# will-rowe/hulk

Hardware: AMD Instinct MI355X
Metric: reads/sec (150bp, k=21, sketch=512) (higher is better)
Workload: dtype u64

## Files before the change

hulk_amd/csrc/hulk_api.hip:

```cpp
#include "hulk_oneshot.h"

#include <mutex>

#include <algorithm>
#include <cmath>
#include <cfloat>

using namespace hulk;

namespace {
thread_local std::string g_create_error;

uint64_t ipow(uint64_t a, uint64_t b) {
    uint64_t p = 1;
    while (b > 0) { if (b & 1) p *= a; b >>= 1; a *= a; }
    return p;
}

}

namespace hulk {
const char *err_text(int status) {
    switch (status) {
        case HULK_OK: return "";
// ... 89 lines not shown
    fq_sweep_idle();
    hulk_ctx *c = new hulk_ctx();
    c->p = p; c->B = (int32_t)bins; c->S = p.sketch_size; c->slot_begin = p.slot_begin; c->slots = p.slot_count;
    c->drift = p.decay_ratio != 1.0;
    c->scaling = p.decay_ratio > 0.0 && p.decay_ratio < 1.0;
    c->decay_weight = c->scaling ? std::exp(-p.decay_ratio) : 0.0;
    c->cms_width = (int)std::ceil(2 / 0.001);
    c->cms_depth = (int)std::ceil(std::log(1 - 0.99) / std::log(0.5));
    c->ntiles = (c->B + SCAN_TILE - 1) / SCAN_TILE;
    c->row_stride = (size_t)c->ntiles * SCAN_TILE;

#define CHK_CREATE(call) do { hipError_t e_ = (call); if (e_ != hipSuccess) { int rc_ = fail_hip(nullptr, e_, #call); hulk_destroy(c); return rc_; } } while (0)
    CHK_CREATE(hipSetDevice(p.device));
    {
        const int ord = lds_order_verified(p.device);
        if (ord < 0) { const int rc_ = fail_hip(nullptr, (hipError_t)(-ord), "LDS atomic-order self-test"); hulk_destroy(c); return rc_; }
        c->lds_order_ok = ord == 1;
        c->cms_chain = !c->lds_order_ok || (p.flags & HULK_FLAG_CMS_CHAIN) != 0;
    }
    CHK_CREATE(create_lane_stream(&c->own_stream, 0));
    c->stream = c->own_stream;
    const size_t B = (size_t)c->B, S = c->S, SL = c->slots;
    CHK_CREATE(dalloc(&c->d_state, 1));
    auto knob = [](const char *name, uint32_t field, uint32_t dflt, uint32_t lo, uint32_t hi) {
        uint32_t v = field ? field : dflt;
        if (const char *e = HULK_EXP_ENV(name)) { const long x = atol(e); if (x >= (long)lo && x <= (long)hi) v = (uint32_t)x; }
        return v;
    };
    c->T = knob("HULK_BATCH", p.batch, SCAN_BATCH_MAX, 1, SCAN_BATCH_MAX);
    const bool decay_on = p.decay_ratio > 0.0 && p.decay_ratio < 1.0;
    c->work_lanes = knob("HULK_WORK_LANES", p.work_lanes, decay_on ? 1 : 2, 1, 2);
    c->host_copy_threads = knob("HULK_HOST_COPY_THREADS", p.host_copy_threads, 4, 1, 32);
    c->no_overlap = (p.flags & HULK_FLAG_NO_OVERLAP) != 0 || HULK_EXP_ENV("HULK_NO_OVERLAP") != nullptr;
    c->shard_full = (p.flags & HULK_FLAG_SHARD_FULL) != 0 || HULK_EXP_ENV("HULK_SHARD_FULL") != nullptr;
    c->ring_n = c->T + 1;
    const size_t T = c->T, RN = c->ring_n;
    CHK_CREATE(dalloc(&c->d_hist, 2 * RN * B));
    {
        int lo = 0, hi = 0;
        CHK_CREATE(hipDeviceGetStreamPriorityRange(&lo, &hi));
        const char *pe = HULK_EXP_ENV("HULK_FLUSH_PRIORITY");
        const int prio = pe ? atoi(pe) : lo;
        CHK_CREATE(hipStreamCreateWithPriority(&c->flush_stream, hipStreamNonBlocking, prio));
    }
    CHK_CREATE(hipEventCreateWithFlags(&c->ev_binned, hipEventDisableTiming));
    CHK_CREATE(hipEventCreateWithFlags(&c->ev_flushed[0], hipEventDisableTiming));
// ... 61 lines not shown
        std::vector<double> w(S ? S : 1, 1.7976931348623157e308);
        CHK_CREATE(hipMemcpy(c->d_weights, w.data(), w.size() * 8, hipMemcpyHostToDevice));
    }
#undef CHK_CREATE
    int rc = build_chains(c);
    if (rc == HULK_OK && p.cws_source == HULK_CWS_GO_COMPAT) rc = generate_tables(c);
    if (rc == HULK_OK) rc = lanes_prereserve(c);
    if (rc == HULK_OK && hipStreamSynchronize(c->stream) != hipSuccess) rc = HULK_ERR_HIP;
    if (rc != HULK_OK) { g_create_error = c->last_error.empty() ? err_text(rc) : c->last_error; hulk_destroy(c); return rc; }
    *out = c;
    return HULK_OK;
}

void hulk_destroy(hulk_ctx *c) {
    if (!c) return;
    if (c->stream) hipStreamSynchronize(c->stream);
    if (c->own_stream) hipStreamSynchronize(c->own_stream);
    if (c->flush_stream) { hipStreamSynchronize(c->flush_stream); hipStreamDestroy(c->flush_stream); }
    if (c->ev_binned) hipEventDestroy(c->ev_binned);
    for (int i = 0; i < 2; i++) if (c->ev_flushed[i]) hipEventDestroy(c->ev_flushed[i]);
    for (auto &pr : c->prof) { hipEventDestroy(pr.a); hipEventDestroy(pr.b); }
    for (auto &m : c->marks) hipEventDestroy(m.e);
    hipFree(c->d_state); hipFree(c->d_hist); hipFree(c->d_hist_tmp);
    hipFree(c->d_meta8); hipFree(c->d_segsum); hipFree(c->d_cbase);
    hipFree(c->d_segadd); hipFree(c->d_segfac); hipFree(c->d_cstart); hipFree(c->d_sege0);
    hipFree(c->d_ctr); hipFree(c->d_pos16); hipFree(c->d_mins); hipFree(c->d_f64); hipFree(c->d_weights);
    hipFree(c->d_blkcnt); hipFree(c->d_eidx); hipFree(c->d_etot); hipFree(c->d_ctrd);
    hipFree(c->d_candA); hipFree(c->d_candB); hipFree(c->d_rcb); hipFree(c->d_rcp32); hipFree(c->d_rmm); hipFree(c->d_k32); hipFree(c->d_tilemin);
    hipFree(c->d_scanmap); hipFree(c->d_scanlist); hipFree(c->d_scanlist_n); hipFree(c->d_slotmin); hipFree(c->d_kmin32); hipFree(c->d_rext); hipFree(c->d_visited); hipFree(c->d_kminslot);
    for (auto &hs : c->hstage) {
        if (hs.ev) hipEventDestroy(hs.ev);
        if (hs.ev1) hipEventDestroy(hs.ev1);
        if (hs.h_bases) hipHostFree(hs.h_bases);
        if (hs.h_off) hipHostFree(hs.h_off);
        hipFree(hs.d_bases); hipFree(hs.d_off);
    }
    hipFree(c->d_min_slots);
    hipFree(c->mh.kmv); hipFree(c->mh.khf); hipFree(c->mh.xmin); hipFree(c->mh.fed); hipFree(c->d_mh_in);
    for (auto &ln : c->lane) {
        if (ln.stream) { hipStreamSynchronize(ln.stream); hipStreamDestroy(ln.stream); }
        hipFree(ln.d_slow_list); hipFree(ln.d_slow_count);
        hulk::MinimizerList &ml = ln.ml;
        hipFree(ml.x); hipFree(ml.slot); hipFree(ml.key); hipFree(ml.cnt); hipFree(ml.off); hipFree(ml.bsum); hipFree(ml.partial);
        hipFree(ml.nib); hipFree(ml.nib_over); hipFree(ml.dmask); hipFree(ml.dsum);
    }
    for (int i = 0; i < 2; i++) if (c->ev_heavy[i]) hipEventDestroy(c->ev_heavy[i]);
// ... 515 lines not shown
```

hulk_amd/csrc/hulk_countmin.hip:

```cpp
#include "hulk_device.h"

#include <math.h>
#include <stdlib.h>
#include <stdio.h>
#include <algorithm>
#include <mutex>

namespace hulk {
namespace {

__global__ __launch_bounds__(256) void k_count_used(const uint32_t *__restrict__ hists, DevState *st,
                                                    FlushBatch fb) {
    __shared__ unsigned red[4];
    const int t = blockIdx.y;
    const uint32_t slot = ring_slot(fb, t);
    if (blockIdx.x == 0 && t == 0 && threadIdx.x < RING_MAX) st->used[fb.parity ^ 1][threadIdx.x] = 0;
    const uint32_t *hist = hists + (size_t)slot * (size_t)fb.num_bins;
    unsigned cnt = 0;
    for (int32_t b = blockIdx.x * blockDim.x + threadIdx.x; b < fb.num_bins; b += gridDim.x * blockDim.x)
        cnt += hist[b] != 0;
    for (int off = 32; off; off >>= 1) cnt += __shfl_xor(cnt, off);
    if (lane_id() == 0) red[threadIdx.x >> 6] = cnt;
    __syncthreads();
    if (threadIdx.x == 0) {
// ... 5 lines not shown
constexpr int CMS_SEGS = 16;
inline int cms_seg_chunks(int32_t num_bins) { return ((num_bins + 63) / 64 + CMS_SEGS - 1) / CMS_SEGS; }

__device__ __forceinline__ void cms_seg_row_sums(uint32_t *lctr, const uint32_t *__restrict__ hist, const uint16_t *__restrict__ pos16,
                                                 size_t B, int64_t b0, int depth, int width, int seg_chunks) {
    const int tid = threadIdx.x, lane = tid & 63, d = tid >> 6;
    for (int i = tid; i < depth * width; i += blockDim.x) lctr[i] = 0;
    __syncthreads();
    if (d >= depth) return;
    const uint16_t *pd = pos16 + (size_t)d * B;
    for (int c0 = 0; c0 < seg_chunks; c0 += 8) {
        uint32_t h[8]; uint32_t p[8];
#pragma unroll
        for (int u = 0; u < 8; u++) {
            const int64_t b = b0 + (int64_t)(c0 + u) * 64 + lane;
            const bool ok = (c0 + u < seg_chunks) && b < (int64_t)B;
            h[u] = ok ? hist[b] : 0u; p[u] = ok ? pd[b] : 0u;
        }
#pragma unroll
        for (int u = 0; u < 8; u++) if (h[u]) atomicAdd(&lctr[d * width + p[u]], h[u]);
    }
}

__global__ __launch_bounds__(512) void k_cms_segsum(const uint32_t *__restrict__ hists,
                                                    const uint16_t *__restrict__ pos16,
                                                    uint32_t *__restrict__ segsum, int depth, int width,
                                                    int seg_chunks, const DevState *st, FlushBatch fb) {
    extern __shared__ __align__(16) unsigned char smem[];
    uint32_t *lctr = (uint32_t *)smem;
    const int seg = blockIdx.x, t = blockIdx.y, tid = threadIdx.x;
    const uint32_t gomask = batch_gomask(st, fb);
    if (!((gomask >> t) & 1u)) return;
    const size_t B = (size_t)fb.num_bins;
    cms_seg_row_sums(lctr, hists + (size_t)ring_slot(fb, t) * B, pos16, B, (int64_t)seg * seg_chunks * 64, depth, width, seg_chunks);
    __syncthreads();
    uint32_t *out = segsum + (((size_t)t * depth) * CMS_SEGS + 0) * width;
    for (int i = tid; i < depth * width; i += blockDim.x) {
        const int dd = i / width, p = i - dd * width;
        out[((size_t)dd * CMS_SEGS + seg) * width + p] = lctr[i];
    }
}

__global__ __launch_bounds__(256) void k_cms_base(const uint32_t *__restrict__ segsum,
                                                  unsigned long long *__restrict__ ctr,
                                                  unsigned long long *__restrict__ base, int depth, int width,
                                                  const DevState *st, FlushBatch fb) {
    const uint32_t gomask = batch_gomask(st, fb);
    const int i = blockIdx.x * blockDim.x + threadIdx.x;
    if (i >= depth * width) return;
    const int d = i / width, p = i - d * width;
    unsigned long long run = ctr[i];
    for (int t = 0; t < (int)fb.count; t++) {
        if (!((gomask >> t) & 1u)) continue;
        uint32_t sv[CMS_SEGS];
        const size_t at0 = (((size_t)t * depth + d) * CMS_SEGS) * width + p;
#pragma unroll
        for (int seg = 0; seg < CMS_SEGS; seg++) sv[seg] = segsum[at0 + (size_t)seg * width];
#pragma unroll
        for (int seg = 0; seg < CMS_SEGS; seg++) { base[at0 + (size_t)seg * width] = run; run += sv[seg]; }
    }
    ctr[i] = run;
}

// ... 369 lines not shown
    const size_t lds3 = (size_t)depth * width * 8 + (size_t)2 * CMS_GB * 8;
    static bool attr_set = false;
    if (!attr_set) {
        hipError_t e = hipFuncSetAttribute((const void *)k_cms_freq, hipFuncAttributeMaxDynamicSharedMemorySize, (int)lds3);
        if (e == hipSuccess) e = hipFuncSetAttribute((const void *)k_cms_freq_chain, hipFuncAttributeMaxDynamicSharedMemorySize, (int)lds3);
        if (e != hipSuccess) return e;
        attr_set = true;
    }
    prof_mark(s, "k_cms_segsum");
    hipLaunchKernelGGL(k_cms_segsum, dim3(CMS_SEGS, fb.count), dim3(512), lds1, s, d_hists, d_pos16, d_segsum, depth, width,
                       seg_chunks, st, fb);
    prof_mark(s, "k_cms_base");
    hipLaunchKernelGGL(k_cms_base, dim3((depth * width + 255) / 256), dim3(256), 0, s, d_segsum, d_ctr, d_base, depth, width, st, fb);
    if (chain) {
        prof_mark(s, "k_cms_freq_chain");
        hipLaunchKernelGGL(k_cms_freq_chain, dim3(CMS_SEGS, fb.count), dim3(512), lds3, s, d_base, d_meta8, d_hists, d_pos16, d_f64,
                           d_rcp32, depth, width, seg_chunks, row_stride, st, fb);
    }
    else {
        prof_mark(s, "k_cms_freq");
        hipLaunchKernelGGL(k_cms_freq, dim3(CMS_SEGS, fb.count), dim3(512), lds3, s, d_base, d_hists, d_pos16, d_f64,
                           d_rcp32, depth, width, seg_chunks, row_stride, st, fb);
    }
    return hipGetLastError();
}

size_t cms_binorder_entries(int depth, int width) { return (size_t)depth * CMS_SEGS * width; }

hipError_t launch_cmsd_binorder(hipStream_t s, uint32_t *d_hists, const uint16_t *d_pos16, const uint8_t *d_meta8,
                                const uint32_t *d_eidx, const uint32_t *d_etot, double *d_ctrd, double *d_segadd,
                                double *d_segfac, uint32_t *d_sege0, double *d_cstart, double *d_f64, float *d_rcp32,
                                int depth, int width, size_t row_stride, double omega, DevState *st, const FlushBatch &fb_in,
                                hipEvent_t freq_begin, hipEvent_t freq_end, bool chain_form) {
    FlushBatch fb = fb_in;
    const int seg_chunks = cms_seg_chunks(fb.num_bins);
    if (depth > 8) return hipErrorInvalidValue;
    { static const char *e = HULK_EXP_ENV("HULK_CMSD_PRIO"); fb.prio = e ? atoi(e) : CMSD_WAVE_PRIO; }
    const size_t lds1 = (size_t)depth * width * 8 + (size_t)2 * 512 * 8;
    const size_t lds3 = (size_t)depth * width * 8 + (size_t)2 * CMS_GB * 8;
    static bool attr_set = false;
    if (!attr_set) {
        hipError_t e = hipFuncSetAttribute((const void *)k_cmsd_segsum, hipFuncAttributeMaxDynamicSharedMemorySize, (int)lds1);
        if (e == hipSuccess) e = hipFuncSetAttribute((const void *)k_cmsd_freq, hipFuncAttributeMaxDynamicSharedMemorySize, (int)lds3);
        if (e == hipSuccess) e = hipFuncSetAttribute((const void *)k_cmsd_freq_chain, hipFuncAttributeMaxDynamicSharedMemorySize, (int)lds3);
        if (e != hipSuccess) return e;
        attr_set = true;
// ... 231 lines not shown
```

hulk_amd/csrc/hulk_ctx.h:

```cpp
#pragma once
#include "../../include/hulk_hip.h"
#include "hulk_internal.h"

#include <rccl/rccl.h>

#include <cstdlib>
#include <cstring>
#include <string>
#include <vector>

static inline int poison_byte() {
    static const int v = [] { const char *e = HULK_EXP_ENV("HULK_POISON"); return e ? (int)(strtol(e, nullptr, 0) & 0xff) : -1; }();
    return v;
}
static inline hipError_t poison_malloc(void **p, size_t n) {
    hipError_t e = (hipMalloc)(p, n);
    if (e == hipSuccess && poison_byte() >= 0 && n) { e = hipMemset(*p, poison_byte(), n); if (e == hipSuccess) e = hipDeviceSynchronize(); }
    return e;
}
static inline hipError_t poison_host_malloc(void **p, size_t n, unsigned flags) {
    hipError_t e = (hipHostMalloc)(p, n, flags);
    if (e == hipSuccess && poison_byte() >= 0 && n) memset(*p, poison_byte(), n);
    return e;
}
// ... 91 lines not shown
    hipEvent_t ev_long = nullptr; hipStream_t long_last_stream = nullptr; bool long_pending = false;
    const uint64_t *h_off_chunk = nullptr;
    uint64_t long_cap = 0, long_table_cap = 0;
    struct Snapshots {
        uint32_t every = 0, cap = 0;
        unsigned long long *d_mins = nullptr; double *d_weights = nullptr;
        uint64_t *h_mins = nullptr; double *h_weights = nullptr;
        std::vector<hulk_snapshot_info> info;
        uint64_t ordinal = 0;
        uint64_t recorded = 0, delivered = 0;
        uint64_t reads_at_flush = 0, reads_at_snapshot = 0;
        hulk_snapshot_fn fn = nullptr; void *user = nullptr; bool fn_failed = false;
        hulk_snapshot_panel_fn pfn = nullptr;
        bool has_fn() const { return fn || pfn; }
        struct Panel {
            uint32_t n = 0; int metric = 0, role = 0;
            double *d_mT = nullptr, *d_wT = nullptr;
            double *d_dist = nullptr, *h_dist = nullptr;
        } panel;
        struct Group { uint64_t first; uint32_t n; hipEvent_t ev; };
        std::vector<Group> groups; size_t group_head = 0;
        std::vector<hipEvent_t> free_events;
    } snap;
    uint64_t seq_count = 0, flush_index = 0;
    uint32_t T = 16, ring_n = 17, ring_base = 0;
    uint32_t bin_spectra = 0;
    bool tables_ready = false, finished = false, hist_hook_used = false;
    int sticky = HULK_OK;
    std::string last_error;
    int profiling = 0;
    std::vector<hulk::ProfileRec> prof;
    std::vector<hulk::ProfMark> marks;
};

namespace hulk {

const char *err_text(int status);
int fail(hulk_ctx *c, int status, const std::string &extra = std::string());
int fail_hip(hulk_ctx *c, hipError_t e, const char *what);
#define HIPCHK(c, call)                                             \
    do { hipError_t e_ = (call); if (e_ != hipSuccess) return hulk::fail_hip((c), e_, #call); } while (0)
template <typename T> hipError_t dalloc(T **p, size_t n) { return hipMalloc((void **)p, n ? n * sizeof(T) : sizeof(T)); }
inline bool metric_ok(int metric) { return metric == HULK_METRIC_JACCARD || metric == HULK_METRIC_WEIGHTED_JACCARD; }
inline bool pair_metric_ok(int metric) { return metric_ok(metric) || metric == HULK_METRIC_BOTTOMK; }
inline bool bottomk_size_ok(int metric, uint32_t sketch_size) { return metric != HULK_METRIC_BOTTOMK || sketch_size <= HULK_MINHASH_MAX_SKETCH; }
inline bool role_ok(int role) { return role == HULK_PANEL_ROW || role == HULK_PANEL_COLUMN; }

int build_chains(hulk_ctx *c);
int install_tables(hulk_ctx *c, const double *r, const double *cc, const double *b);
int generate_tables(hulk_ctx *c);
int ensure_tables(hulk_ctx *c);

constexpr unsigned PROFILE_EVENT_FLAGS = hipEventDisableSystemFence;
uint32_t *ring_hist(hulk_ctx *c);
int issue_flush(hulk_ctx *c, hipEvent_t gate = nullptr);
int ring_issue_own_flush(hulk_ctx *c);
hipEvent_t ring_write_event(hulk_ctx *c);
int ring_ready_for_writes(hulk_ctx *c);
int sync_all(hulk_ctx *c);
int fatal_status(hulk_ctx *c);
int bin_reads(hulk_ctx *c, const uint8_t *d_bases, const uint64_t *d_offsets, uint64_t n,
              uint32_t max_len, uint64_t bases_bytes, uint64_t interval, uint64_t fill, bool join = false);
hipStream_t lane_stream(hulk_ctx *c, int ring);
hipStream_t ring_stream(hulk_ctx *c);
int lanes_join(hulk_ctx *c);
int lanes_prereserve(hulk_ctx *c);
int stage_mark_busy(hulk_ctx *c, hulk_ctx::HostStage &hs);
int flush_kernels(hulk_ctx *c, hipStream_t s, uint32_t *hist, const FlushBatch &fb);
bool no_overlap_mode(const hulk_ctx *c);
hipStream_t flush_stream_of(hulk_ctx *c);
enum { FLUSH_EXPLICIT = 0, FLUSH_INTERVAL = 1, FLUSH_EOF = 2 };
int flush_batch(hulk_ctx *c, uint32_t count, hipStream_t dep_stream = nullptr, bool use_dep = false, bool allreduce = false,
                int closed_by = FLUSH_EXPLICIT);
int check_device_error(hulk_ctx *c);
int stage_host_reads(hulk_ctx *c, const uint8_t *bases, const uint64_t *offsets, uint64_t i0, uint64_t i1,
                     hulk_ctx::HostStage **out);
int check_host_reads(hulk_ctx *c, const uint64_t *offsets, uint64_t n, uint64_t *max_len_out);

hipError_t create_lane_stream(hipStream_t *s, int priority);
struct ProfScope {
    hulk_ctx *prev;
    explicit ProfScope(hulk_ctx *c);
    ~ProfScope();
};

int snap_plan(hulk_ctx *c, FlushBatch &fb, uint32_t count, int closed_by, uint64_t *first, uint32_t *n);
int snap_flush_issued(hulk_ctx *c, hipStream_t s, uint64_t first, uint32_t n);
int snap_deliver(hulk_ctx *c, bool wait, uint32_t *delivered = nullptr);
void snap_teardown(hulk_ctx *c);
int snap_panel_flush(hulk_ctx *c, hipStream_t s, const FlushBatch &fb);
int snap_refuse(hulk_ctx *c, const char *entry);
// ... 6 lines not shown
```

hulk_amd/csrc/hulk_cws.hip:

```cpp
#include "hulk_device.h"

#include <math.h>
#include <stdlib.h>
#include <algorithm>

namespace hulk {
namespace {

__device__ __forceinline__ float wave_min8_by_row(float (&m)[8]) {
    asm volatile("s_nop 1\n\t"
                 "v_permlane32_swap_b32 %0, %4\n\t"
                 "v_permlane32_swap_b32 %1, %5\n\t"
                 "v_permlane32_swap_b32 %2, %6\n\t"
                 "v_permlane32_swap_b32 %3, %7\n\t"
                 "v_min_f32 %0, %0, %4\n\t"
                 "v_min_f32 %2, %2, %6\n\t"
                 "v_min_f32 %1, %1, %5\n\t"
                 "v_min_f32 %3, %3, %7\n\t"
                 "v_permlane16_swap_b32 %0, %2\n\t"
                 "s_nop 0\n\t"
                 "v_permlane16_swap_b32 %1, %3\n\t"
                 "v_min_f32 %0, %0, %2\n\t"
                 "v_min_f32 %1, %1, %3\n\t"
                 "s_nop 1\n\t"
                 "v_min_f32_dpp %0, %0, %0 row_ror:8 row_mask:0xf bank_mask:0xf\n\t"
                 "v_min_f32_dpp %1, %1, %1 row_ror:8 row_mask:0xf bank_mask:0xf\n\t"
                 "s_nop 1\n\t"
                 "v_mov_b32_dpp %0, %1 quad_perm:[0,1,2,3] row_mask:0xf bank_mask:0xc\n\t"
                 "s_nop 1\n\t"
                 "v_min_f32_dpp %0, %0, %0 quad_perm:[1,0,3,2] row_mask:0xf bank_mask:0xf\n\t"
                 "s_nop 1\n\t"
                 "v_min_f32_dpp %0, %0, %0 quad_perm:[2,3,0,1] row_mask:0xf bank_mask:0xf\n\t"
                 "s_nop 1\n\t"
                 "v_min_f32_dpp %0, %0, %0 row_half_mirror row_mask:0xf bank_mask:0xf\n\t"
                 : "+v"(m[0]), "+v"(m[1]), "+v"(m[2]), "+v"(m[3]), "+v"(m[4]), "+v"(m[5]), "+v"(m[6]), "+v"(m[7]));
    return m[0];
}

__global__ __launch_bounds__(1024) void k_flush_decide(const unsigned long long *__restrict__ ctr, int ncounters,
                                                       const float *__restrict__ kminslot,
                                                       const double *__restrict__ weights, int slots, int slot_begin,
                                                       DevState *st, FlushBatch fb, int enable,
                                                       unsigned long long *seal, uint32_t seal_tag) {
    __shared__ unsigned long long red[16];
    __shared__ int anypass;
    const int tid = threadIdx.x;
    if (tid == 0) anypass = 0;
    unsigned long long m = ~0ull;
    for (int i = tid; i < ncounters; i += blockDim.x) { const unsigned long long v = ctr[i]; m = v < m ? v : m; }
    for (int off = 32; off; off >>= 1) { const unsigned long long o = __shfl_xor(m, off); m = o < m ? o : m; }
    if ((tid & 63) == 0) red[tid >> 6] = m;
    __syncthreads();
    m = red[0];
    for (int i = 1; i < 16; i++) m = red[i] < m ? red[i] : m;
    bool pass = false;
    if (enable == 2) pass = false;
    else if (!enable || m == 0) pass = true;
    else {
        const double rmax = 1.0 / (double)m;
        for (int s = tid; s < slots; s += blockDim.x) {
            const double km = (double)kminslot[s];
            const double w = weights[slot_begin + s];
            const double thr = w + 1e-5 * fabs(w) + 1e-37;
            const double bound = km < 0.0 ? km * rmax : 0.0;
            if (bound <= thr) pass = true;
        }
    }
    if (pass) atomicOr(&anypass, 1);
    __syncthreads();
    if (tid == 0) {
        if (seal) *seal = ((unsigned long long)seal_tag << 32) | (anypass ? 1ull : 0ull);
        else st->skip_exact[fb.parity] = anypass ? 0u : 1u;
    }
}
__global__ __launch_bounds__(256) void k_slot_kmin(const float *__restrict__ kmin32, float *__restrict__ kminslot, int wtiles) {
    __shared__ float red[4];
    const int slot = blockIdx.x;
    float m = INFINITY;
    for (int i = threadIdx.x; i < wtiles; i += blockDim.x) m = fminf(m, kmin32[(size_t)slot * wtiles + i]);
    for (int off = 32; off; off >>= 1) m = fminf(m, __shfl_xor(m, off));
    if ((threadIdx.x & 63) == 0) red[threadIdx.x >> 6] = m;
    __syncthreads();
    if (threadIdx.x == 0) kminslot[slot] = fminf(fminf(red[0], red[1]), fminf(red[2], red[3]));
}

__global__ __launch_bounds__(256) void k_tile_kmin(const float *__restrict__ k32, float *__restrict__ kmin32,
                                                   int ntiles, size_t row_stride) {
    const int slot = blockIdx.y, tile = blockIdx.x, wid = threadIdx.x >> 6;
    const floatx4 v = *(const floatx4 *)(k32 + (size_t)slot * row_stride + (size_t)tile * SCAN_TILE + (size_t)threadIdx.x * 4);
    float m = fminf(fminf(v.x, v.y), fminf(v.z, v.w));
    for (int off = 32; off; off >>= 1) m = fminf(m, __shfl_xor(m, off));
    if ((threadIdx.x & 63) == 0) kmin32[(size_t)slot * (size_t)(ntiles * 4) + (size_t)(tile * 4 + wid)] = m;
}
__global__ __launch_bounds__(256) void k_rcp_extrema(const float *__restrict__ rcp32, float *__restrict__ rext,
                                                     int ntiles, size_t row_stride, const DevState *st, FlushBatch fb) {
// ... 675 lines not shown
    if (grid_form) {
        const dim3 g((unsigned)(((wwords * 4 + 7) / 8) * 8 * groups));
        if (mode == 0) { prof_mark(s, "k_cws_scan"); hipLaunchKernelGGL(k_cws_scan<0>, g, dim3(1024), 0, s, d_k32, rv, d_tilemin, slots, ntiles, row_stride, st, fb, d_scanmap, wwords); }
        else if (mode == 1) { prof_mark(s, "k_cws_scan"); hipLaunchKernelGGL(k_cws_scan<1>, g, dim3(1024), 0, s, d_k32, rv, d_tilemin, slots, ntiles, row_stride, st, fb, d_scanmap, wwords); }
        else { prof_mark(s, "k_cws_scan"); hipLaunchKernelGGL(k_cws_scan<2>, g, dim3(1024), 0, s, d_k32, rv, d_tilemin, slots, ntiles, row_stride, st, fb, d_scanmap, wwords); }
    } else {
        const size_t items = (size_t)groups * wtiles;
        const dim3 g((unsigned)((std::min<size_t>(2048, (items + 3) / 4) + 7) / 8 * 8));
        if (mode == 0) { prof_mark(s, "k_cws_scan_list"); hipLaunchKernelGGL(k_cws_scan_list<0>, g, dim3(256), 0, s, d_k32, rv, d_tilemin, slots, ntiles, row_stride, st, fb, d_scanlist, d_scanlist_n); }
        else if (mode == 1) { prof_mark(s, "k_cws_scan_list"); hipLaunchKernelGGL(k_cws_scan_list<1>, g, dim3(256), 0, s, d_k32, rv, d_tilemin, slots, ntiles, row_stride, st, fb, d_scanlist, d_scanlist_n); }
        else { prof_mark(s, "k_cws_scan_list"); hipLaunchKernelGGL(k_cws_scan_list<2>, g, dim3(256), 0, s, d_k32, rv, d_tilemin, slots, ntiles, row_stride, st, fb, d_scanlist, d_scanlist_n); }
    }
    if (scan_end) { const hipError_t e = hipEventRecord(scan_end, s); if (e != hipSuccess) return e; }
    return hipGetLastError();
}

hipError_t launch_slot_kmin(hipStream_t s, const float *d_kmin32, float *d_kminslot, int slots, int ntiles) {
    hipLaunchKernelGGL(k_slot_kmin, dim3(slots), dim3(256), 0, s, d_kmin32, d_kminslot, ntiles * 4);
    return hipGetLastError();
}

hipError_t launch_flush_decide(hipStream_t s, const unsigned long long *d_ctr, int ncounters, const float *d_kminslot,
                               const double *d_weights, int slots, int slot_begin, DevState *st, const FlushBatch &fb,
                               int enable, unsigned long long *d_seal, uint32_t seal_tag) {
    prof_mark(s, "k_flush_decide");
    hipLaunchKernelGGL(k_flush_decide, dim3(1), dim3(1024), 0, s, d_ctr, ncounters, d_kminslot, d_weights, slots,
                       slot_begin, st, fb, enable, d_seal, seal_tag);
    return hipGetLastError();
}

hipError_t launch_tile_kmin(hipStream_t s, const float *d_k32, float *d_kmin32, int slots, int ntiles, size_t row_stride) {
    hipLaunchKernelGGL(k_tile_kmin, dim3(ntiles, slots), dim3(256), 0, s, d_k32, d_kmin32, ntiles, row_stride);
    return hipGetLastError();
}

hipError_t launch_cws_resolve(hipStream_t s, const double *d_rcb, const double *d_f64,
                              const float *d_tilemin, double *d_candA, int32_t *d_candB,
                              unsigned long long *d_mins, double *d_weights,
                              int slots, int slot_begin, int ntiles, const unsigned long long *d_scanmap, DevState *st,
                              const FlushBatch &fb, unsigned long long *d_snap_mins, double *d_snap_weights, uint32_t sketch_size) {
    const int merged = (scan_merge_off() || d_snap_mins) ? 0 : 1;
    if (merged) {
        prof_mark(s, "k_cws_resolve");
        hipLaunchKernelGGL(k_cws_resolve<true>, dim3(slots, 1), dim3(256), (size_t)ntiles * 4 * sizeof(float), s,
                           d_rcb, d_f64, d_tilemin, d_candA, d_candB, slots, ntiles, d_scanmap, (ntiles * 4 + 63) / 64, st, fb);
    }
    else {
        prof_mark(s, "k_cws_resolve");
        hipLaunchKernelGGL(k_cws_resolve<false>, dim3(slots, fb.count), dim3(256), (size_t)ntiles * 4 * sizeof(float), s,
                           d_rcb, d_f64, d_tilemin, d_candA, d_candB, slots, ntiles, d_scanmap, (ntiles * 4 + 63) / 64, st, fb);
// ... 89 lines not shown
```

hulk_amd/csrc/hulk_flush.hip:

```cpp
#include "hulk_ctx.h"

#include <algorithm>
#include <thread>

namespace hulk {

namespace { thread_local hulk_ctx *g_prof_ctx = nullptr; }
ProfScope::ProfScope(hulk_ctx *c) : prev(g_prof_ctx) { g_prof_ctx = (c && (c->profiling & 16)) ? c : nullptr; }
ProfScope::~ProfScope() { g_prof_ctx = prev; }
void prof_mark(hipStream_t s, const char *kernel) {
    hulk_ctx *c = g_prof_ctx;
    if (!c) return;
    ProfMark m{nullptr, kernel, s};
    if (hipEventCreateWithFlags(&m.e, PROFILE_EVENT_FLAGS) != hipSuccess) return;
    if (hipEventRecord(m.e, s) != hipSuccess) { (void)hipEventDestroy(m.e); return; }
    c->marks.push_back(m);
}

hipError_t create_lane_stream(hipStream_t *s, int priority) {
    if (const char *e = HULK_EXP_ENV("HULK_K1_CU_FREE")) {
        const int nfree = atoi(e);
        if (nfree > 0 && nfree < 256) {
            uint32_t mask[8];
            for (int i = 0; i < 8; i++) mask[i] = 0xffffffffu;
// ... 13 lines not shown
static int lane_of_ring(const hulk_ctx *c, int ring) { return (c->work_lanes > 1 && !c->no_overlap) ? ring : 0; }
hipStream_t ring_stream(hulk_ctx *c) { return lane_stream(c, lane_of_ring(c, c->cur_ring)); }

int ring_issue_own_flush(hulk_ctx *c) {
    if (c->deferred.armed && c->deferred.ring == c->cur_ring) return issue_flush(c, nullptr);
    return HULK_OK;
}
hipEvent_t ring_write_event(hulk_ctx *c) {
    if (!c->pending_flush[c->cur_ring]) return nullptr;
    c->pending_flush[c->cur_ring] = false;
    return c->ev_flushed[c->cur_ring];
}
int ring_ready_for_writes(hulk_ctx *c) {
    { const int rc = ring_issue_own_flush(c); if (rc != HULK_OK) return rc; }
    if (hipEvent_t e = ring_write_event(c)) HIPCHK(c, hipStreamWaitEvent(ring_stream(c), e, 0));
    return HULK_OK;
}

int fatal_status(hulk_ctx *c) {
    if (c->sticky == HULK_ERR_HIP || c->sticky == HULK_ERR_COMM) return fail(c, c->sticky);
    return HULK_OK;
}

int sync_all(hulk_ctx *c) {
    { const int rc = fatal_status(c); if (rc != HULK_OK) return rc; }
    { const int rc = issue_flush(c, nullptr); if (rc != HULK_OK) return rc; }
    HIPCHK(c, hipStreamSynchronize(c->stream));
    if (c->lane[1].stream) HIPCHK(c, hipStreamSynchronize(c->lane[1].stream));
    c->stagger = 1;
    HIPCHK(c, hipStreamSynchronize(c->flush_stream));
    return HULK_OK;
}

constexpr uint32_t GENERIC_XCAP_MAX = 1024;
bool pick_config(uint32_t k, uint32_t max_len, MinimizerParams &P, int &threads) {
    const uint32_t npos = max_len >= k ? max_len - k + 1 : 1;
    if (npos <= 192) { P.xcap = 192; P.tab_size = 256; threads = 256; return true; }
    P.xcap = GENERIC_XCAP_MAX; P.tab_size = 2048; threads = 64;
    return npos <= GENERIC_XCAP_MAX;
}

int bin_long_reads(hulk_ctx *c, hipStream_t s, const uint8_t *d_bases, const uint64_t *d_offsets, uint64_t n, MinimizerParams P,
                   uint32_t *hist, const uint64_t *h_offsets) {
    std::vector<uint64_t> fetched;
    const uint64_t *off = h_offsets;
    if (!off) {
        fetched.resize(n + 1);
        HIPCHK(c, hipMemcpyAsync(fetched.data(), d_offsets, (n + 1) * 8, hipMemcpyDeviceToHost, s));
        HIPCHK(c, hipStreamSynchronize(s));
        off = fetched.data();
    }
    constexpr uint64_t GROUP_POS = 128ull << 20;
    constexpr uint32_t GROUP_SEQS = 32768;
// ... 233 lines not shown
        ProfScope prof_scope(c);
        struct Close { hipStream_t s; ~Close() { prof_mark(s, "-"); } } prof_close{s};
        rc = issue_flush(c, nullptr);
        if (rc == HULK_OK) {
            if (hipEvent_t e = ring_write_event(c)) HIPCHK(c, hipStreamWaitEvent(s, e, 0));
            const bool fits = pick_config(c->p.k, max_len, P, threads);
            P.skip_long = fits ? 0u : 1u;
            HIPCHK(c, launch_minimizer_bin(s, d_bases, d_offsets, n, P, threads, hist, c->d_state,
                                           c->d_min_slots, nullptr, nullptr, 0, &c->mh));
            if (!fits) rc = bin_long_reads(c, s, d_bases, d_offsets, n, P, hist, c->h_off_chunk);
        }
    }
    if (rc != HULK_OK) return rc;
    if (li && (join || c->stream != c->own_stream)) return lanes_join(c);
    return HULK_OK;
}

int flush_kernels(hulk_ctx *c, hipStream_t s, uint32_t *hist, const FlushBatch &fb) {
    ProfScope prof_scope(c);
    struct Close { hipStream_t s; ~Close() { prof_mark(s, "-"); } } prof_close{s};
    if (!c->scaling) HIPCHK(c, launch_count_used(s, hist, c->d_state, fb));
    {
        HIPCHK(c, launch_flush_decide(s, c->d_ctr, c->cms_depth * c->cms_width, c->d_kminslot, c->d_weights, (int)c->slots,
                                      (int)c->slot_begin, c->d_state, fb, (c->prune && !c->drift && !c->no_skip && c->slots) ? 1 : 0));
    }
    if (c->scaling) {
        HIPCHK(c, launch_elem_index(s, hist, c->d_blkcnt, c->d_eidx, c->d_etot, fb, c->d_state));
        ProfileRec pf{}; pf.which = 4;
        if ((c->profiling & 8)) { HIPCHK(c, hipEventCreateWithFlags(&pf.a, PROFILE_EVENT_FLAGS)); HIPCHK(c, hipEventCreateWithFlags(&pf.b, PROFILE_EVENT_FLAGS)); }
        HIPCHK(c, launch_cmsd_binorder(s, hist, c->d_pos16, c->d_meta8, c->d_eidx, c->d_etot, c->d_ctrd, c->d_segadd,
                                       c->d_segfac, c->d_sege0, c->d_cstart, c->d_f64, c->d_rcp32, c->cms_depth,
                                       c->cms_width, c->row_stride, c->decay_weight, c->d_state, fb, pf.a, pf.b, c->cms_chain));
        if ((c->profiling & 8)) c->prof.push_back(pf);
        if (HULK_EXP_ENV("HULK_C3_GATE")) {
            c->heavy_idx ^= 1;
            if (!c->ev_heavy[c->heavy_idx]) HIPCHK(c, hipEventCreateWithFlags(&c->ev_heavy[c->heavy_idx], hipEventDisableTiming));
            HIPCHK(c, hipEventRecord(c->ev_heavy[c->heavy_idx], s));
            c->heavy_set[c->heavy_idx] = true;
        }
    } else {
        HIPCHK(c, launch_cms_binorder(s, hist, c->d_pos16, c->d_meta8, c->d_ctr, c->d_segsum, c->d_cbase, c->d_f64,
                                      c->d_rcp32, c->cms_depth, c->cms_width, c->row_stride, c->d_state, fb, c->cms_chain));
    }
    if (c->slots) {
        ProfileRec pr{};
        if ((c->profiling & 1)) { HIPCHK(c, hipEventCreateWithFlags(&pr.a, PROFILE_EVENT_FLAGS)); HIPCHK(c, hipEventCreateWithFlags(&pr.b, PROFILE_EVENT_FLAGS)); }
        HIPCHK(c, launch_cws_scan(s, c->d_k32, c->d_rcp32, c->d_tilemin, (int)c->slots, c->ntiles,
// ... 12 lines not shown
                                     (int)c->slots, (int)c->slot_begin, c->ntiles, c->d_scanmap, c->d_state, fb,
                                     c->snap.d_mins, c->snap.d_weights, c->S));
    }
    if (fb.snap_mask && c->snap.panel.n) { const int rc = snap_panel_flush(c, s, fb); if (rc != HULK_OK) return rc; }
    return HULK_OK;
}

bool no_overlap_mode(const hulk_ctx *c) { return c->no_overlap; }
hipStream_t flush_stream_of(hulk_ctx *c) { return c->no_overlap ? c->stream : c->flush_stream; }

int issue_flush(hulk_ctx *c, hipEvent_t gate) {
    if (!c->deferred.armed) return HULK_OK;
    c->deferred.armed = false;
    const FlushBatch fb = c->deferred.fb;
    const int ring = c->deferred.ring;
    hipStream_t s = flush_stream_of(c);
    if (!no_overlap_mode(c) || c->deferred.use_dep) HIPCHK(c, hipStreamWaitEvent(s, c->ev_binned, 0));
    if (!no_overlap_mode(c) && gate) HIPCHK(c, hipStreamWaitEvent(s, gate, 0));
    uint32_t *hist = c->d_hist + (size_t)ring * (size_t)c->ring_n * (size_t)c->B;
    if (c->deferred.allreduce) {
        const int rc = comm_allreduce_u32(c, s, hist + (size_t)fb.ring_base * (size_t)c->B, (size_t)fb.count * (size_t)c->B);
        if (rc != HULK_OK) return rc;
    }
    { const int rc = flush_kernels(c, s, hist, fb); if (rc != HULK_OK) return rc; }
    if (c->deferred.snap_n) { const int rc = snap_flush_issued(c, s, c->deferred.snap_first, c->deferred.snap_n); if (rc != HULK_OK) return rc; }
    HIPCHK(c, hipEventRecord(c->ev_flushed[ring], s));
    c->pending_flush[ring] = true;
    return HULK_OK;
}

int flush_batch(hulk_ctx *c, uint32_t count, hipStream_t dep_stream, bool use_dep, bool allreduce, int closed_by) {
    { const int rcf = fatal_status(c); if (rcf != HULK_OK) return rcf; }
    if (count == 0) return HULK_OK;
    int rc = ensure_tables(c);
    if (rc != HULK_OK) return rc;
    rc = issue_flush(c);
    if (rc != HULK_OK) return rc;
    FlushBatch fb{};
    fb.ring_base = c->ring_base; fb.ring_n = c->ring_n; fb.count = count;
    fb.parity = (int)(c->flush_index & 1); fb.num_bins = c->B;
    uint64_t snap_first = 0; uint32_t snap_n = 0;
    if (c->snap.every) { rc = snap_plan(c, fb, count, closed_by, &snap_first, &snap_n); if (rc != HULK_OK) return rc; }
    HIPCHK(c, hipEventRecord(c->ev_binned, use_dep ? dep_stream : ring_stream(c)));
    c->deferred.armed = true; c->deferred.fb = fb; c->deferred.ring = c->cur_ring;
    c->deferred.use_dep = use_dep; c->deferred.allreduce = allreduce;
    c->deferred.snap_first = snap_first; c->deferred.snap_n = snap_n;
// ... 119 lines not shown
```

hulk_amd/csrc/hulk_internal.h:

```cpp
#pragma once
#include <hip/hip_runtime.h>
#include <stdint.h>
#include <stdlib.h>
#include <chrono>

#ifdef HULK_EXPERIMENTS
#define HULK_EXP_ENV(name) getenv(name)
#else
#define HULK_EXP_ENV(name) ((const char *)nullptr)
#endif

namespace hulk {

constexpr int CMS_DEPTH_MAX = 8;
constexpr int SCAN_TILE = 1024;
constexpr int SCAN_ROWS = 8;
constexpr int SCAN_BATCH_MAX = 16;
constexpr int RING_MAX = SCAN_BATCH_MAX + 1;
constexpr int MIN_SLOTS = 8192;

struct DevState {
    unsigned long long total_len;
    unsigned long long n_elements;
    unsigned int used[2][RING_MAX];
// ... 73 lines not shown
hipError_t launch_minimizer_bin(hipStream_t s, const uint8_t *d_bases, const uint64_t *d_offsets,
                                uint64_t n_reads, MinimizerParams P, int block_threads,
                                uint32_t *d_hist, DevState *d_state, unsigned long long *d_min_slots,
                                const uint32_t *d_read_list, const uint32_t *d_read_list_count,
                                uint32_t list_blocks, const MinHashState *mh = nullptr);
hipError_t launch_minimizer_fast(hipStream_t s, const uint8_t *d_bases, const uint64_t *d_offsets,
                                 uint64_t n_reads, MinimizerParams P, const MinimizerList &ml,
                                 DevState *d_state, unsigned long long *d_min_slots);
hipError_t launch_minimizer_post(hipStream_t s, uint64_t n_reads, MinimizerParams P, const MinimizerList &ml,
                                 uint32_t *d_hists, uint32_t *d_slow_list, uint32_t *d_slow_count,
                                 hipEvent_t jump_begin = nullptr, hipEvent_t jump_end = nullptr,
                                 hipEvent_t wait_before_spectra = nullptr, uint32_t *geom = nullptr);
constexpr int SPECTRUM_GEOM_WORDS = 5;
uint32_t minimizer_list_rcap(uint32_t w, bool pair);
hipError_t launch_long_group(hipStream_t s, const uint8_t *d_bases, const LongSeqDesc *d_desc, uint32_t n_seqs,
                             uint64_t max_npos, MinimizerParams P, uint64_t *d_xs, uint8_t *d_valid, uint64_t *d_table,
                             uint64_t table_total, uint32_t *d_hists, unsigned long long *d_min_slots);
hipError_t launch_count_used(hipStream_t s, const uint32_t *d_hists, DevState *st, const FlushBatch &fb);
hipError_t launch_build_chains(hipStream_t s, uint16_t *d_pos16, uint8_t *d_meta8, int32_t num_bins, int depth, int width);
hipError_t launch_cms_binorder(hipStream_t s, uint32_t *d_hists, const uint16_t *d_pos16, const uint8_t *d_meta8,
                               unsigned long long *d_ctr, uint32_t *d_segsum, unsigned long long *d_base,
                               double *d_f64, float *d_rcp32, int depth, int width, size_t row_stride,
                               DevState *st, const FlushBatch &fb, bool chain = false);
int lds_order_verified(int device);
size_t cms_binorder_entries(int depth, int width);
hipError_t launch_cmsd_binorder(hipStream_t s, uint32_t *d_hists, const uint16_t *d_pos16, const uint8_t *d_meta8,
                                const uint32_t *d_eidx, const uint32_t *d_etot, double *d_ctrd, double *d_segadd,
                                double *d_segfac, uint32_t *d_sege0, double *d_cstart, double *d_f64, float *d_rcp32,
                                int depth, int width, size_t row_stride, double omega, DevState *st, const FlushBatch &fb,
                                hipEvent_t freq_begin = nullptr, hipEvent_t freq_end = nullptr, bool chain_form = false);
hipError_t launch_cws_scan(hipStream_t s, const float *d_k32, const float *d_rcp32, float *d_tilemin,
                           int slots, int ntiles, size_t row_stride, DevState *st, const FlushBatch &fb,
                           const float *d_kmin32, float *d_rext, const double *d_weights, int slot_begin,
                           unsigned long long *d_visited, double drift_dw, unsigned long long *d_scanmap, bool per_interval,
                           float *d_rmm, uint32_t *d_scanlist, uint32_t *d_scanlist_n, hipEvent_t scan_begin = nullptr,
                           hipEvent_t scan_end = nullptr);
hipError_t launch_tile_kmin(hipStream_t s, const float *d_k32, float *d_kmin32, int slots, int ntiles, size_t row_stride);
hipError_t launch_slot_kmin(hipStream_t s, const float *d_kmin32, float *d_kminslot, int slots, int ntiles);
hipError_t launch_flush_decide(hipStream_t s, const unsigned long long *d_ctr, int ncounters, const float *d_kminslot,
                               const double *d_weights, int slots, int slot_begin, DevState *st, const FlushBatch &fb,
                               int enable, unsigned long long *d_seal = nullptr, uint32_t seal_tag = 0);
constexpr int SHARD_HDR = 32;
constexpr int SHARD_VERDICT = 0, SHARD_TAG = 1, SHARD_USED = 2;
hipError_t launch_shard_check(hipStream_t s, const uint32_t *d_hdr_all, uint32_t world, uint32_t step_tag, DevState *st,
                              uint32_t *h_out, int fatal);
hipError_t launch_shard_local(hipStream_t s, uint32_t *d_hists, const uint16_t *d_pos16, uint32_t *d_hdr, uint32_t *d_delta,
                              int depth, int width, const FlushBatch &fb);
hipError_t launch_shard_apply(hipStream_t s, const uint32_t *d_hdr_all, const uint32_t *d_delta_all, unsigned long long *d_ctr,
                              int depth, int width, uint32_t world, uint32_t T, uint32_t step_intervals, int32_t num_bins,
                              DevState *st, uint32_t step_tag);
hipError_t launch_cws_resolve(hipStream_t s, const double *d_rcb, const double *d_f64,
                              const float *d_tilemin, double *d_candA, int32_t *d_candB,
                              unsigned long long *d_mins, double *d_weights,
                              int slots, int slot_begin, int ntiles, const unsigned long long *d_scanmap, DevState *st,
                              const FlushBatch &fb, unsigned long long *d_snap_mins = nullptr, double *d_snap_weights = nullptr,
                              uint32_t sketch_size = 0);
hipError_t launch_elem_index(hipStream_t s, const uint32_t *d_hists, uint32_t *d_blkcnt, uint32_t *d_eidx,
                             uint32_t *d_etot, const FlushBatch &fb, DevState *st);
int elem_index_blocks(int32_t num_bins);
hipError_t launch_cws_resolve_drift(hipStream_t s, const double *d_rcb, const double *d_f64,
                                    const float *d_tilemin, unsigned long long *d_mins, double *d_weights,
                                    int slots, int slot_begin, int ntiles, double decay_weight, float *d_slotmin,
                                    const unsigned long long *d_scanmap, DevState *st, const FlushBatch &fb,
                                    unsigned long long *d_snap_mins = nullptr, double *d_snap_weights = nullptr,
// ... 52 lines not shown
```

hulk_amd/csrc/hulk_tables.hip:

```cpp
#include "hulk_ctx.h"
#include "cws_gen.h"
#include "go_rng_jump.h"

#include <algorithm>
#include <cmath>

namespace hulk {
namespace {
int32_t jump_host(uint64_t key, int64_t n) {
    int64_t b = -1, j = 0;
    if (n <= 0) n = 1;
    while (j < n) {
        b = j;
        key = key * 2862933555777941757ull + 1;
        j = (int64_t)((double)(b + 1) * ((double)(1LL << 31) / (double)((key >> 33) + 1)));
    }
    return (int32_t)b;
}

}

int build_chains(hulk_ctx *c) {
    const int D = c->cms_depth, W = c->cms_width; const int32_t B = c->B;
    if (!HULK_EXP_ENV("HULK_CHAINS_HOST")) {
// ... 12 lines not shown
            pos16[(size_t)d * B + b] = (uint16_t)pos[b];
        }
        std::vector<int32_t> last_bin(W, -1);
        for (int32_t c0 = 0; c0 < B; c0 += 64) {
            const int32_t c1 = std::min<int32_t>(B, c0 + 64);
            for (int32_t b = c0; b < c1; b++) {
                const int32_t prev = last_bin[pos[b]];
                uint8_t m = 64;
                if (prev >= c0) { m = (uint8_t)(prev - c0); meta8[(size_t)d * B + prev] &= 0x7f; }
                meta8[(size_t)d * B + b] = m | 0x80;
                last_bin[pos[b]] = b;
            }
        }
    }
    HIPCHK(c, dalloc(&c->d_meta8, meta8.size()));
    HIPCHK(c, hipMemcpy(c->d_meta8, meta8.data(), meta8.size(), hipMemcpyHostToDevice));
    HIPCHK(c, dalloc(&c->d_pos16, pos16.size()));
    HIPCHK(c, hipMemcpy(c->d_pos16, pos16.data(), pos16.size() * 2, hipMemcpyHostToDevice));
    return HULK_OK;
}

int install_tables(hulk_ctx *c, const double *r, const double *cc, const double *b) {
    const size_t B = (size_t)c->B;
    std::vector<double> row(B * 3);
    for (uint32_t s = 0; s < c->slots; s++) {
        const size_t src = (size_t)(c->slot_begin + s) * B;
        for (size_t j = 0; j < B; j++) { row[j * 3] = r[src + j]; row[j * 3 + 1] = cc[src + j]; row[j * 3 + 2] = b[src + j]; }
        HIPCHK(c, hipMemcpy(c->d_rcb + (size_t)s * B * 3, row.data(), B * 3 * sizeof(double), hipMemcpyHostToDevice));
    }
    HIPCHK(c, launch_build_k32(c->stream, c->d_rcb, c->d_k32, (int)c->slots, c->B, c->row_stride));
    if (c->slots) {
        HIPCHK(c, launch_tile_kmin(c->stream, c->d_k32, c->d_kmin32, (int)c->slots, c->ntiles, c->row_stride));
        HIPCHK(c, launch_slot_kmin(c->stream, c->d_kmin32, c->d_kminslot, (int)c->slots, c->ntiles));
    }
    c->tables_ready = true;
    return HULK_OK;
}

int generate_tables_host(hulk_ctx *c) {
    const uint64_t B = (uint64_t)c->B;
    const uint64_t need_entries = (uint64_t)(c->slot_begin + c->slots) * B;
    if (need_entries == 0) { c->tables_ready = true; return HULK_OK; }
    const uint64_t need_gammas = 2 * need_entries;
    const size_t CH = (size_t)1 << 22;
    const CwsConstants K((c->p.flags & HULK_FLAG_GAMMA_CPYTHON) != 0);
    uint64_t *h_buf[2] = {nullptr, nullptr}; uint64_t *d_pairs[2] = {nullptr, nullptr};
// ... 145 lines not shown
        GEN_CHK(launch_tile_kmin(c->stream, c->d_k32, c->d_kmin32, (int)c->slots, c->ntiles, c->row_stride));
        GEN_CHK(launch_slot_kmin(c->stream, c->d_kmin32, c->d_kminslot, (int)c->slots, c->ntiles));
    }
    GEN_CHK(hipStreamSynchronize(c->stream));
#undef GEN_CHK
    cleanup();
    c->tables_ready = true;
    return HULK_OK;
}

int generate_tables(hulk_ctx *c) {
    static const bool host_only = HULK_EXP_ENV("HULK_CWS_HOST") != nullptr;
    if (!host_only) {
        const int rc = generate_tables_device(c);
        if (rc <= 0) return rc;
    }
    return generate_tables_host(c);
}

int ensure_tables(hulk_ctx *c) {
    if (c->tables_ready) return HULK_OK;
    if (c->p.cws_source == HULK_CWS_EXTERNAL)
        return fail(c, HULK_ERR_STATE, "cws_source is EXTERNAL but hulk_set_cws_tables was not called");
    return generate_tables(c);
}

}
```

Baseline: 2.085 billion.

## Add steady-state flush path that skips exact CWS work once pruning is proven

The flush-decide kernel now publishes its skip verdict, tagged with a flush counter, to a mapped host word. Once the host sees a positive verdict, later flushes take a steady path. That path runs only the count-min segment sums, zeroes the histograms and adds into the counters, skipping the elem-index, scan and CWS kernels. The device re-checks skip_exact and raises an error if the proof no longer holds. This is meant to cut per-flush kernel count and scan work, at the cost of extra host/device verdict plumbing and reset logic when tables change.

```diff
diff --git a/hulk_amd/csrc/hulk_api.hip b/hulk_amd/csrc/hulk_api.hip
--- a/hulk_amd/csrc/hulk_api.hip
+++ b/hulk_amd/csrc/hulk_api.hip
@@ -135,6 +135,8 @@
     c->stream = c->own_stream;
     const size_t B = (size_t)c->B, S = c->S, SL = c->slots;
     CHK_CREATE(dalloc(&c->d_state, 1));
+    CHK_CREATE(hipHostMalloc((void **)&c->h_verdict, 8, hipHostMallocMapped));
+    *c->h_verdict = 0;
     auto knob = [](const char *name, uint32_t field, uint32_t dflt, uint32_t lo, uint32_t hi) {
         uint32_t v = field ? field : dflt;
         if (const char *e = HULK_EXP_ENV(name)) { const long x = atol(e); if (x >= (long)lo && x <= (long)hi) v = (uint32_t)x; }
@@ -242,6 +244,7 @@
     for (auto &pr : c->prof) { hipEventDestroy(pr.a); hipEventDestroy(pr.b); }
     for (auto &m : c->marks) hipEventDestroy(m.e);
     hipFree(c->d_state); hipFree(c->d_hist); hipFree(c->d_hist_tmp);
+    if (c->h_verdict) hipHostFree(c->h_verdict);
     hipFree(c->d_meta8); hipFree(c->d_segsum); hipFree(c->d_cbase);
     hipFree(c->d_segadd); hipFree(c->d_segfac); hipFree(c->d_cstart); hipFree(c->d_sege0);
     hipFree(c->d_ctr); hipFree(c->d_pos16); hipFree(c->d_mins); hipFree(c->d_f64); hipFree(c->d_weights);
diff --git a/hulk_amd/csrc/hulk_countmin.hip b/hulk_amd/csrc/hulk_countmin.hip
--- a/hulk_amd/csrc/hulk_countmin.hip
+++ b/hulk_amd/csrc/hulk_countmin.hip
@@ -51,23 +51,76 @@
     }
 }
 
-__global__ __launch_bounds__(512) void k_cms_segsum(const uint32_t *__restrict__ hists,
-                                                    const uint16_t *__restrict__ pos16,
-                                                    uint32_t *__restrict__ segsum, int depth, int width,
-                                                    int seg_chunks, const DevState *st, FlushBatch fb) {
+template <bool STEADY, class Hist>
+__device__ __forceinline__ void cms_segsum(Hist *__restrict__ hists, const uint16_t *__restrict__ pos16,
+                                           uint32_t *__restrict__ segsum, int depth, int width, int seg_chunks,
+                                           const DevState *st, const FlushBatch &fb) {
     extern __shared__ __align__(16) unsigned char smem[];
     uint32_t *lctr = (uint32_t *)smem;
     const int seg = blockIdx.x, t = blockIdx.y, tid = threadIdx.x;
     const uint32_t gomask = batch_gomask(st, fb);
     if (!((gomask >> t) & 1u)) return;
+    if (STEADY && !st->skip_exact[fb.parity]) return;
     const size_t B = (size_t)fb.num_bins;
-    cms_seg_row_sums(lctr, hists + (size_t)ring_slot(fb, t) * B, pos16, B, (int64_t)seg * seg_chunks * 64, depth, width, seg_chunks);
+    Hist *hist = hists + (size_t)ring_slot(fb, t) * B;
+    const int64_t b0 = (int64_t)seg * seg_chunks * 64;
+    cms_seg_row_sums(lctr, hist, pos16, B, b0, depth, width, seg_chunks);
     __syncthreads();
     uint32_t *out = segsum + (((size_t)t * depth) * CMS_SEGS + 0) * width;
     for (int i = tid; i < depth * width; i += blockDim.x) {
         const int dd = i / width, p = i - dd * width;
         out[((size_t)dd * CMS_SEGS + seg) * width + p] = lctr[i];
     }
+    if constexpr (STEADY) {
+        const int64_t w1 = b0 + (int64_t)seg_chunks * 64;
+        for (int64_t b = b0 + tid; b < w1 && b < (int64_t)B; b += blockDim.x) hist[b] = 0;
+    }
+}
+__global__ __launch_bounds__(512) void k_cms_segsum(const uint32_t *__restrict__ hists,
+                                                    const uint16_t *__restrict__ pos16,
+                                                    uint32_t *__restrict__ segsum, int depth, int width,
+                                                    int seg_chunks, const DevState *st, FlushBatch fb) {
+    cms_segsum<false>(hists, pos16, segsum, depth, width, seg_chunks, st, fb);
+}
+
+__global__ __launch_bounds__(512) void k_cms_steady_sums(uint32_t *__restrict__ hists, const uint16_t *__restrict__ pos16,
+                                                         uint32_t *__restrict__ segsum, int depth, int width,
+                                                         int seg_chunks, const DevState *st, FlushBatch fb) {
+    cms_segsum<true>(hists, pos16, segsum, depth, width, seg_chunks, st, fb);
+}
+
+__global__ __launch_bounds__(256) void k_cms_steady_add(const uint32_t *__restrict__ segsum,
+                                                        unsigned long long *__restrict__ ctr, int depth, int width,
+                                                        DevState *st, FlushBatch fb) {
+    const uint32_t gomask = batch_gomask(st, fb);
+    const bool proven = st->skip_exact[fb.parity] != 0u;
+    const int i = blockIdx.x * blockDim.x + threadIdx.x;
+    if (i == 0) {
+        if (!proven) set_error(st, -34);
+        else {
+            unsigned long long elems = 0; bool few = false;
+            for (int t = 0; t < (int)fb.count; t++) {
+                const unsigned used = st->used[fb.parity][ring_slot(fb, t)];
+                if ((gomask >> t) & 1u) elems += used;
+                else if (used != 0) few = true;
+            }
+            if (few) set_error(st, -5);
+            if (elems) atomicAdd(&st->n_elements, elems);
+        }
+    }
+    if (!proven || i >= depth * width) return;
+    const int d = i / width, p = i - d * width;
+    unsigned long long sum = 0;
+    for (int t = 0; t < (int)fb.count; t++) {
+        if (!((gomask >> t) & 1u)) continue;
+        uint32_t sv[CMS_SEGS];
+        const size_t at0 = (((size_t)t * depth + d) * CMS_SEGS) * width + p;
+#pragma unroll
+        for (int seg = 0; seg < CMS_SEGS; seg++) sv[seg] = segsum[at0 + (size_t)seg * width];
+#pragma unroll
+        for (int seg = 0; seg < CMS_SEGS; seg++) sum += sv[seg];
+    }
+    if (sum) ctr[i] += sum;
 }
 
 __global__ __launch_bounds__(256) void k_cms_base(const uint32_t *__restrict__ segsum,
@@ -483,6 +536,16 @@
         hipLaunchKernelGGL(k_cms_freq, dim3(CMS_SEGS, fb.count), dim3(512), lds3, s, d_base, d_hists, d_pos16, d_f64,
                            d_rcp32, depth, width, seg_chunks, row_stride, st, fb);
     }
+    return hipGetLastError();
+}
+
+hipError_t launch_cms_steady(hipStream_t s, uint32_t *d_hists, const uint16_t *d_pos16, unsigned long long *d_ctr,
+                             uint32_t *d_segsum, int depth, int width, DevState *st, const FlushBatch &fb) {
+    prof_mark(s, "k_cms_steady_sums");
+    hipLaunchKernelGGL(k_cms_steady_sums, dim3(CMS_SEGS, fb.count), dim3(512), (size_t)depth * width * 4, s, d_hists, d_pos16,
+                       d_segsum, depth, width, cms_seg_chunks(fb.num_bins), st, fb);
+    prof_mark(s, "k_cms_steady_add");
+    hipLaunchKernelGGL(k_cms_steady_add, dim3((depth * width + 255) / 256), dim3(256), 0, s, d_segsum, d_ctr, depth, width, st, fb);
     return hipGetLastError();
 }
 
diff --git a/hulk_amd/csrc/hulk_ctx.h b/hulk_amd/csrc/hulk_ctx.h
--- a/hulk_amd/csrc/hulk_ctx.h
+++ b/hulk_amd/csrc/hulk_ctx.h
@@ -137,6 +137,9 @@
         std::vector<Group> groups; size_t group_head = 0;
         std::vector<hipEvent_t> free_events;
     } snap;
+    unsigned long long *h_verdict = nullptr;
+    bool steady = false;
+    uint32_t flush_tag = 0, steady_tag_min = 1;
     uint64_t seq_count = 0, flush_index = 0;
     uint32_t T = 16, ring_n = 17, ring_base = 0;
     uint32_t bin_spectra = 0;
@@ -182,6 +185,8 @@
 int lanes_prereserve(hulk_ctx *c);
 int stage_mark_busy(hulk_ctx *c, hulk_ctx::HostStage &hs);
 int flush_kernels(hulk_ctx *c, hipStream_t s, uint32_t *hist, const FlushBatch &fb);
+bool steady_eligible(const hulk_ctx *c);
+void steady_reset(hulk_ctx *c);
 bool no_overlap_mode(const hulk_ctx *c);
 hipStream_t flush_stream_of(hulk_ctx *c);
 enum { FLUSH_EXPLICIT = 0, FLUSH_INTERVAL = 1, FLUSH_EOF = 2 };
diff --git a/hulk_amd/csrc/hulk_cws.hip b/hulk_amd/csrc/hulk_cws.hip
--- a/hulk_amd/csrc/hulk_cws.hip
+++ b/hulk_amd/csrc/hulk_cws.hip
@@ -41,7 +41,8 @@
                                                        const float *__restrict__ kminslot,
                                                        const double *__restrict__ weights, int slots, int slot_begin,
                                                        DevState *st, FlushBatch fb, int enable,
-                                                       unsigned long long *seal, uint32_t seal_tag) {
+                                                       unsigned long long *seal, uint32_t seal_tag,
+                                                       unsigned long long *h_verdict, uint32_t flush_tag) {
     __shared__ unsigned long long red[16];
     __shared__ int anypass;
     const int tid = threadIdx.x;
@@ -70,7 +71,10 @@
     __syncthreads();
     if (tid == 0) {
         if (seal) *seal = ((unsigned long long)seal_tag << 32) | (anypass ? 1ull : 0ull);
-        else st->skip_exact[fb.parity] = anypass ? 0u : 1u;
+        else {
+            st->skip_exact[fb.parity] = anypass ? 0u : 1u;
+            if (h_verdict) { __builtin_nontemporal_store(verdict_word(flush_tag, !anypass), h_verdict); __threadfence_system(); }
+        }
     }
 }
 __global__ __launch_bounds__(256) void k_slot_kmin(const float *__restrict__ kmin32, float *__restrict__ kminslot, int wtiles) {
@@ -792,10 +796,11 @@
 
 hipError_t launch_flush_decide(hipStream_t s, const unsigned long long *d_ctr, int ncounters, const float *d_kminslot,
                                const double *d_weights, int slots, int slot_begin, DevState *st, const FlushBatch &fb,
-                               int enable, unsigned long long *d_seal, uint32_t seal_tag) {
+                               int enable, unsigned long long *d_seal, uint32_t seal_tag, unsigned long long *h_verdict,
+                               uint32_t flush_tag) {
     prof_mark(s, "k_flush_decide");
     hipLaunchKernelGGL(k_flush_decide, dim3(1), dim3(1024), 0, s, d_ctr, ncounters, d_kminslot, d_weights, slots,
-                       slot_begin, st, fb, enable, d_seal, seal_tag);
+                       slot_begin, st, fb, enable, d_seal, seal_tag, h_verdict, flush_tag);
     return hipGetLastError();
 }
 
diff --git a/hulk_amd/csrc/hulk_flush.hip b/hulk_amd/csrc/hulk_flush.hip
--- a/hulk_amd/csrc/hulk_flush.hip
+++ b/hulk_amd/csrc/hulk_flush.hip
@@ -59,6 +59,22 @@
     return HULK_OK;
 }
 
+bool steady_eligible(const hulk_ctx *c) {
+    return c->prune && !c->drift && !c->scaling && !c->no_skip && c->slots && !c->snap.every && !c->snap.panel.n &&
+           !c->comm.kind && !c->deferred.allreduce && !HULK_EXP_ENV("HULK_NO_STEADY_FLUSH");
+}
+static void steady_adopt(hulk_ctx *c) {
+    if (c->steady || !c->h_verdict || !steady_eligible(c)) return;
+    const unsigned long long w = __atomic_load_n(c->h_verdict, __ATOMIC_RELAXED);
+    const uint32_t tag = (uint32_t)(w >> 32);
+    if ((w & 1ull) && tag >= c->steady_tag_min && tag <= c->flush_tag) c->steady = true;
+}
+void steady_reset(hulk_ctx *c) {
+    c->steady = false;
+    c->steady_tag_min = c->flush_tag + 1;
+    if (c->h_verdict) __atomic_store_n(c->h_verdict, 0ull, __ATOMIC_RELAXED);
+}
+
 int sync_all(hulk_ctx *c) {
     { const int rc = fatal_status(c); if (rc != HULK_OK) return rc; }
     { const int rc = issue_flush(c, nullptr); if (rc != HULK_OK) return rc; }
@@ -66,6 +82,7 @@
     if (c->lane[1].stream) HIPCHK(c, hipStreamSynchronize(c->lane[1].stream));
     c->stagger = 1;
     HIPCHK(c, hipStreamSynchronize(c->flush_stream));
+    steady_adopt(c);
     return HULK_OK;
 }
 
@@ -345,7 +362,13 @@
     if (!c->scaling) HIPCHK(c, launch_count_used(s, hist, c->d_state, fb));
     {
         HIPCHK(c, launch_flush_decide(s, c->d_ctr, c->cms_depth * c->cms_width, c->d_kminslot, c->d_weights, (int)c->slots,
-                                      (int)c->slot_begin, c->d_state, fb, (c->prune && !c->drift && !c->no_skip && c->slots) ? 1 : 0));
+                                      (int)c->slot_begin, c->d_state, fb, (c->prune && !c->drift && !c->no_skip && c->slots) ? 1 : 0,
+                                      nullptr, 0, c->h_verdict, ++c->flush_tag));
+    }
+    if (c->steady && steady_eligible(c)) {
+        HIPCHK(c, launch_cms_steady(s, hist, c->d_pos16, c->d_ctr, c->d_segsum, c->cms_depth, c->cms_width, c->d_state, fb));
+        c->scan_tiles_total += (uint64_t)((c->slots + SCAN_ROWS - 1) / SCAN_ROWS) * (uint64_t)c->ntiles * 4u;
+        return HULK_OK;
     }
     if (c->scaling) {
         HIPCHK(c, launch_elem_index(s, hist, c->d_blkcnt, c->d_eidx, c->d_etot, fb, c->d_state));
@@ -404,6 +427,7 @@
         const int rc = comm_allreduce_u32(c, s, hist + (size_t)fb.ring_base * (size_t)c->B, (size_t)fb.count * (size_t)c->B);
         if (rc != HULK_OK) return rc;
     }
+    if (!no_overlap_mode(c)) steady_adopt(c);
     { const int rc = flush_kernels(c, s, hist, fb); if (rc != HULK_OK) return rc; }
     if (c->deferred.snap_n) { const int rc = snap_flush_issued(c, s, c->deferred.snap_first, c->deferred.snap_n); if (rc != HULK_OK) return rc; }
     HIPCHK(c, hipEventRecord(c->ev_flushed[ring], s));
diff --git a/hulk_amd/csrc/hulk_internal.h b/hulk_amd/csrc/hulk_internal.h
--- a/hulk_amd/csrc/hulk_internal.h
+++ b/hulk_amd/csrc/hulk_internal.h
@@ -119,6 +119,8 @@
                                unsigned long long *d_ctr, uint32_t *d_segsum, unsigned long long *d_base,
                                double *d_f64, float *d_rcp32, int depth, int width, size_t row_stride,
                                DevState *st, const FlushBatch &fb, bool chain = false);
+hipError_t launch_cms_steady(hipStream_t s, uint32_t *d_hists, const uint16_t *d_pos16, unsigned long long *d_ctr,
+                             uint32_t *d_segsum, int depth, int width, DevState *st, const FlushBatch &fb);
 int lds_order_verified(int device);
 size_t cms_binorder_entries(int depth, int width);
 hipError_t launch_cmsd_binorder(hipStream_t s, uint32_t *d_hists, const uint16_t *d_pos16, const uint8_t *d_meta8,
@@ -136,7 +138,9 @@
 hipError_t launch_slot_kmin(hipStream_t s, const float *d_kmin32, float *d_kminslot, int slots, int ntiles);
 hipError_t launch_flush_decide(hipStream_t s, const unsigned long long *d_ctr, int ncounters, const float *d_kminslot,
                                const double *d_weights, int slots, int slot_begin, DevState *st, const FlushBatch &fb,
-                               int enable, unsigned long long *d_seal = nullptr, uint32_t seal_tag = 0);
+                               int enable, unsigned long long *d_seal = nullptr, uint32_t seal_tag = 0,
+                               unsigned long long *h_verdict = nullptr, uint32_t flush_tag = 0);
+__host__ __device__ inline unsigned long long verdict_word(uint32_t flush_tag, bool skip) { return ((unsigned long long)flush_tag << 32) | (skip ? 1ull : 0ull); }
 constexpr int SHARD_HDR = 32;
 constexpr int SHARD_VERDICT = 0, SHARD_TAG = 1, SHARD_USED = 2;
 hipError_t launch_shard_check(hipStream_t s, const uint32_t *d_hdr_all, uint32_t world, uint32_t step_tag, DevState *st,
diff --git a/hulk_amd/csrc/hulk_tables.hip b/hulk_amd/csrc/hulk_tables.hip
--- a/hulk_amd/csrc/hulk_tables.hip
+++ b/hulk_amd/csrc/hulk_tables.hip
@@ -58,6 +58,7 @@
 
 int install_tables(hulk_ctx *c, const double *r, const double *cc, const double *b) {
     const size_t B = (size_t)c->B;
+    steady_reset(c);
     std::vector<double> row(B * 3);
     for (uint32_t s = 0; s < c->slots; s++) {
         const size_t src = (size_t)(c->slot_begin + s) * B;
@@ -249,6 +250,7 @@
     if (c->tables_ready) return HULK_OK;
     if (c->p.cws_source == HULK_CWS_EXTERNAL)
         return fail(c, HULK_ERR_STATE, "cws_source is EXTERNAL but hulk_set_cws_tables was not called");
+    steady_reset(c);
     return generate_tables(c);
 }
 
```

After: 2.169 billion (median of 6 runs). 1.04x the previous value.
